# gotzmann/llama.go

Measured on AMD Instinct MI355X. Metric: decode tokens/s LLaMA-7B fp32; % HBM-read roofline, higher is better.
Workload: dtype f32

## Files before the change

llama.go_amd/csrc/kernels_common.h:

```cpp
#pragma once
#include <hip/hip_runtime.h>
#include <stdint.h>

namespace lh {

typedef float f4 __attribute__((ext_vector_type(4)));
typedef float f2 __attribute__((ext_vector_type(2)));
typedef unsigned int u4 __attribute__((ext_vector_type(4)));

struct StepParams {
    uint32_t token;
    uint32_t past;
    uint32_t step;
    uint32_t pad;
};

struct BatchRow {
    float* kc;
    float* vc;
    uint32_t pos;
    uint32_t step;
};

__device__ __forceinline__ f4 ld_nt(const f4* p) { return __builtin_nontemporal_load(p); }
// ... 31 lines not shown
}
__device__ __forceinline__ double wave_sum_f64(double v) {
#pragma unroll
    for (int o = 32; o >= 1; o >>= 1) v += __shfl_xor(v, o, 64);
    return v;
}

__device__ __forceinline__ void wg_row_block(uint32_t M, uint32_t wg_q, uint32_t wg_r, uint32_t* r0, uint32_t* r1) {
    const uint32_t b = blockIdx.x, nwg = gridDim.x;
    if (wg_q | wg_r) {
        *r0 = 2u * (b * wg_q + (b < wg_r ? b : wg_r));
        *r1 = (b + 1 == nwg) ? M : 2u * ((b + 1) * wg_q + (b + 1 < wg_r ? b + 1 : wg_r));
    } else {
        const uint32_t npairs = M >> 1;
        *r0 = 2u * (uint32_t)(((uint64_t)b * npairs) / nwg);
        *r1 = (b + 1 == nwg) ? M : 2u * (uint32_t)(((uint64_t)(b + 1) * npairs) / nwg);
    }
}

#define LH_TOUCH_ARGS(...) do { lh::touch_args_(__VA_ARGS__); } while (0)
template <typename A, typename B> __device__ __forceinline__ void touch_args_(A a, B b) { asm volatile("" ::"s"(a), "s"(b)); }
template <typename A, typename B, typename C> __device__ __forceinline__ void touch_args_(A a, B b, C c) { asm volatile("" ::"s"(a), "s"(b), "s"(c)); }
template <typename A, typename B, typename C, typename D> __device__ __forceinline__ void touch_args_(A a, B b, C c, D d) { asm volatile("" ::"s"(a), "s"(b), "s"(c), "s"(d)); }
template <typename A, typename B, typename C, typename D, typename E, typename F> __device__ __forceinline__ void touch_args_(A a, B b, C c, D d, E e, F f) {
    asm volatile("" ::"s"(a), "s"(b), "s"(c), "s"(d), "s"(e), "s"(f));
}

__device__ __forceinline__ const char* sgpr_ptr(const void* p) {
    uint32_t lo = (uint32_t)(uintptr_t)p, hi = (uint32_t)((uintptr_t)p >> 32);
    lo = __builtin_amdgcn_readfirstlane(lo);
    hi = __builtin_amdgcn_readfirstlane(hi);
    asm volatile("" : "+s"(lo), "+s"(hi));
    return (const char*)(((uintptr_t)hi << 32) | lo);
}

__device__ __forceinline__ float silu_ref(float x) {
    const float den = (float)(1.0 + exp((double)(-x)));
    return __fdiv_rn(x, den);
}
__device__ __forceinline__ void rope_rotate(float x0f, float x1f, double2 cs, float* o0, float* o1) {
    const double x0 = (double)x0f, x1 = (double)x1f;
    *o0 = (float)__dsub_rn(__dmul_rn(x0, cs.x), __dmul_rn(x1, cs.y));
    *o1 = (float)__dadd_rn(__dmul_rn(x0, cs.y), __dmul_rn(x1, cs.x));
}

__device__ __forceinline__ void split3(float x, uint32_t* hi, uint32_t* mid, uint32_t* lo) {
// ... 12 lines not shown
```

llama.go_amd/csrc/kernels_llama.h:

```cpp
#pragma once
#include "kernels_common.h"

namespace lh {

enum { PRO_PLAIN = 0, PRO_RMSNORM = 1 };
enum { EPI_STORE = 0, EPI_RESID = 1, EPI_QKV_ROPE = 2, EPI_SILU_MUL = 3 };
enum { MAP_SINGLE = 0, MAP_BLOCK = 1, MAP_PAIR = 2 };

struct GemvArgs {
    const float* w[3];
    const float* ws[3];
    uint32_t rows_per_mat;
    uint32_t M;
    uint32_t K;
    const float* x;
    const float* gamma;
    float* y;
    const float* resid;
    float* q_out;
    float* k_cache;
    float* v_cache;
    const double2* rope;
    uint32_t hd;
    uint32_t d;
    const StepParams* sp;
    uint32_t wg_q, wg_r;
};

template <int KI, int TH>
__device__ __forceinline__ void rmsnorm_prologue(f4 (&xr)[KI], const bool (&act)[KI], const f4 (&gr)[KI], uint32_t K, double* sred) {
    constexpr int NW = TH / 64;
    const int tid = threadIdx.x, lane = tid & 63, wave = tid >> 6;
    double s = 0.0;
#pragma unroll
    for (int j = 0; j < KI; ++j) {
        if (act[j]) {
            s += (double)__fmul_rn(xr[j].x, xr[j].x);
            s += (double)__fmul_rn(xr[j].y, xr[j].y);
            s += (double)__fmul_rn(xr[j].z, xr[j].z);
            s += (double)__fmul_rn(xr[j].w, xr[j].w);
        }
    }
    s = wave_sum_f64(s);
    if (lane == 0) sred[wave] = s;
    __syncthreads();
    double tot = 0.0;
#pragma unroll
    for (int w = 0; w < NW; ++w) tot += sred[w];
    const double mean = tot / (double)K;
    const float scale = (float)(1.0 / sqrt(mean + 1e-5));
#pragma unroll
    for (int j = 0; j < KI; ++j) {
        if (act[j]) {
            const f4 g = gr[j];
            xr[j].x = __fmul_rn(g.x, __fmul_rn(xr[j].x, scale));
            xr[j].y = __fmul_rn(g.y, __fmul_rn(xr[j].y, scale));
            xr[j].z = __fmul_rn(g.z, __fmul_rn(xr[j].z, scale));
            xr[j].w = __fmul_rn(g.w, __fmul_rn(xr[j].w, scale));
        }
    }
}

template <int EPI, int NP>
__device__ __forceinline__ void gemv_finish(const GemvArgs& a, const float* red, uint32_t r0, uint32_t r1, uint32_t fin, float resid_pre,
                                            double2 cs_pre, uint32_t past_pre) {
    if (r0 + fin >= r1) return;
    const float* p0 = red + fin * NP;
    float s0 = 0.f;
#pragma unroll
    for (int k = 0; k < NP; ++k) s0 += p0[k];
    const uint32_t v = r0 + fin;
    if (EPI == EPI_STORE) {
        a.y[v] = s0;
    } else if (EPI == EPI_RESID) {
        a.y[v] = __fadd_rn(s0, resid_pre);
    } else {
        const float* p1 = p0 + NP;
        float s1 = 0.f;
#pragma unroll
        for (int k = 0; k < NP; ++k) s1 += p1[k];
        if (EPI == EPI_SILU_MUL) {
            a.y[v >> 1] = __fmul_rn(silu_ref(s0), s1);
        } else {
            const uint32_t d = a.d;
// ... 24 lines not shown
    } else if (EPI == EPI_QKV_ROPE) {
        *past_pre = a.sp->past;
        const uint32_t v = r0 + fin;
        if (v < r1 && v < 2 * a.d) {
            const uint32_t e = v < a.d ? v : v - a.d;
            *cs_pre = a.rope[(size_t)*past_pre * (a.hd >> 1) + ((e % a.hd) >> 1)];
        }
    }
}

template <int MAP>
__device__ __forceinline__ const char* gemv_row_base(const char* w0, const char* w1, const char* w2, uint32_t rows_per_mat, uint32_t v, uint64_t row_bytes) {
    if (MAP == MAP_SINGLE) return w0 + (uint64_t)v * row_bytes;
    if (MAP == MAP_BLOCK) {
        const uint32_t m = (v >= rows_per_mat ? 1u : 0u) + (v >= 2u * rows_per_mat ? 1u : 0u);
        const char* b = m == 0 ? w0 : (m == 1 ? w1 : w2);
        return b + (uint64_t)(v - m * rows_per_mat) * row_bytes;
    }
    return ((v & 1u) ? w1 : w0) + (uint64_t)(v >> 1) * row_bytes;
}

template <int KI, int U, int TH, int PRO, int EPI, int MAP>
__global__ __launch_bounds__(TH) void k_gemv_sa(const GemvArgs a) {
    LH_TOUCH_ARGS(a.w[0], a.x, a.hd, a.wg_r);
    extern __shared__ __attribute__((aligned(16))) char smem_raw[];
    constexpr int NW = TH / 64;
    double* sred = (double*)smem_raw;
    float* red = (float*)(smem_raw + NW * 8);
    const int tid = threadIdx.x, lane = tid & 63, wave = tid >> 6;
    const uint32_t K4 = a.K >> 2;
    uint32_t r0, r1;
    wg_row_block(a.M, a.wg_q, a.wg_r, &r0, &r1);
    const char *w0 = (const char*)a.w[0], *w1 = (const char*)a.w[1], *w2 = (const char*)a.w[2];
    const char* xdummy = (const char*)a.x;
    const uint32_t rpm = a.rows_per_mat;
    const uint64_t row_bytes = (uint64_t)a.K * 4;

    const uint32_t fin = (EPI == EPI_STORE || EPI == EPI_RESID) ? (uint32_t)tid : 2u * (uint32_t)tid;
    float resid_pre;
    double2 cs_pre;
    uint32_t past_pre;
    gemv_prefetch_fin<EPI>(a, r0, r1, fin, &resid_pre, &cs_pre, &past_pre);
    f4 xr[KI];
    f4 gr[KI];
    bool act[KI];
    uint32_t loff[KI];
#pragma unroll
    for (int j = 0; j < KI; ++j) {
        act[j] = (uint32_t)(tid + j * TH) < K4;
        loff[j] = act[j] ? (uint32_t)(tid + j * TH) * 16u : 0u;
        xr[j] = act[j] ? ((const f4*)a.x)[tid + j * TH] : f4{0.f, 0.f, 0.f, 0.f};
        if (PRO == PRO_RMSNORM) gr[j] = act[j] ? ((const f4*)a.gamma)[tid + j * TH] : f4{0.f, 0.f, 0.f, 0.f};
    }
    f4 w[U][KI];
#pragma unroll
    for (int u = 0; u < U; ++u) {
        const char* p = (r0 + u < r1) ? gemv_row_base<MAP>(w0, w1, w2, rpm, r0 + u, row_bytes) : xdummy;
#pragma unroll
        for (int j = 0; j < KI; ++j) w[u][j] = ld_nt((const f4*)(p + loff[j]));
    }
    if (PRO == PRO_RMSNORM) rmsnorm_prologue<KI, TH>(xr, act, gr, a.K, sred);
    for (uint32_t r = r0; r < r1; r += U) {
        float acc[U];
#pragma unroll
        for (int u = 0; u < U; ++u) {
            const uint32_t nr = r + U + u;
            const char* p = nr < r1 ? gemv_row_base<MAP>(w0, w1, w2, rpm, nr, row_bytes) : xdummy;
            float s = 0.f;
#pragma unroll
            for (int j = 0; j < KI; ++j) {
                const f4 c = w[u][j];
                s = fmaf(c.x, xr[j].x, s);
                s = fmaf(c.y, xr[j].y, s);
                s = fmaf(c.z, xr[j].z, s);
                s = fmaf(c.w, xr[j].w, s);
                w[u][j] = ld_nt((const f4*)(p + loff[j]));
            }
            acc[u] = s;
        }
#pragma unroll
        for (int u = 0; u < U; ++u) acc[u] = wave_sum(acc[u]);
        if (lane == 0) {
#pragma unroll
            for (int u = 0; u < U; ++u)
// ... 234 lines not shown
    for (uint32_t t0 = ph + VP * phases; t0 < T; t0 += VP * phases) {
        float vv[VP];
#pragma unroll
        for (int i = 0; i < VP; ++i) {
            const uint32_t t = t0 + (uint32_t)i * phases;
            vv[i] = Vc[(size_t)(t < T ? t : 0) * d + c];
        }
#pragma unroll
        for (int i = 0; i < VP; ++i) {
            const uint32_t t = t0 + (uint32_t)i * phases;
            if (t < T) acc = fmaf(vv[i], __fmul_rn(pr[t], inv), acc);
        }
    }
    scratch[tid] = acc;
    __syncthreads();
    if (tid < (int)hd) {
        float o = scratch[tid];
        for (uint32_t p2 = 1; p2 < phases; ++p2) o += scratch[tid + p2 * hd];
        a.out[(size_t)j * d + h * hd + tid] = o;
        if (a.out_s3) attn_store_split3(a, (size_t)j * d + h * hd + tid, o);
    }
}

constexpr int ATT_TC = 128;

__global__ __launch_bounds__(ATT_TH) void k_attention_split(const AttnArgs a, float* __restrict__ part) {
    LH_TOUCH_ARGS(a.q, a.sp, a.rows);
    __shared__ float sc[ATT_TC];
    __shared__ float pr[ATT_TC];
    __shared__ float scratch[ATT_TH];
    constexpr int NG = ATT_TH / 32;
    const int tid = threadIdx.x, lane = tid & 63;
    const uint32_t h = blockIdx.x, ch = blockIdx.y, nch = gridDim.y, j = blockIdx.z;
    const uint32_t past = a.rows ? a.rows[j].pos : (a.sp ? a.sp->past : a.past_host);
    const uint32_t T = past + 1, c0 = ch * ATT_TC;
    if (c0 >= T) return;
    const uint32_t Tl = (T - c0 < (uint32_t)ATT_TC) ? T - c0 : (uint32_t)ATT_TC;
    const uint32_t d = a.d, hd = a.hd;
    const float* q = a.q + (size_t)j * d + h * hd;
    typedef const float __attribute__((address_space(1))) gfl;
    typedef const f4 __attribute__((address_space(1))) gf4;
    gfl* Kc = (gfl*)(uintptr_t)((a.rows ? a.rows[j].kc + a.kv_off : a.k_cache) + (size_t)c0 * d + h * hd);
    gfl* Vc = (gfl*)(uintptr_t)((a.rows ? a.rows[j].vc + a.kv_off : a.v_cache) + (size_t)c0 * d + h * hd);
    const uint32_t phases = ATT_TH / hd, c = tid % hd, ph = tid / hd;
    constexpr int VP = ATT_TC / 8;
    float vpre[VP];
#pragma unroll
    for (int i = 0; i < VP; ++i) {
// ... 312 lines not shown
```

llama.go_amd/csrc/kernels_q8.h:

```cpp
#pragma once
#include "kernels_llama.h"

namespace lh {

__device__ __forceinline__ u4 ld_nt_u4(const u4* p) { return __builtin_nontemporal_load(p); }


__device__ __forceinline__ float dot16_q8(const u4 q, const f4 (&x)[4]) {
    f2 a0 = {0.f, 0.f}, a1 = {0.f, 0.f};
#pragma unroll
    for (int k = 0; k < 4; ++k) {
        const int d = (int)q[k];
        const f2 w0 = {(float)(int)(signed char)(d), (float)(int)(signed char)(d >> 8)};
        const f2 w1 = {(float)(int)(signed char)(d >> 16), (float)(d >> 24)};
        a0 = __builtin_elementwise_fma(w0, f2{x[k].x, x[k].y}, a0);
        a1 = __builtin_elementwise_fma(w1, f2{x[k].z, x[k].w}, a1);
    }
    return (a0.x + a0.y) + (a1.x + a1.y);
}

template <int KI, int U, int TPR, int PRO, int EPI, int MAP, int TH = 1024>
__global__ __launch_bounds__(TH) void k_gemv_q8s(const GemvArgs a) {
    LH_TOUCH_ARGS(a.w[0], a.x, a.hd, a.wg_r);
    extern __shared__ __attribute__((aligned(16))) char smem_raw[];
    constexpr int G = TH / TPR, NWR = TPR / 64;
    static_assert(TPR % 64 == 0, "a row group must be a whole number of waves");
    double* sred = (double*)smem_raw;
    float* red = (float*)(smem_raw + 16 * 8);
    const int tid = threadIdx.x, lane = tid & 63, wave = tid >> 6;
    const int tr = tid % TPR, wr = wave % NWR;
    const uint32_t grp = (uint32_t)__builtin_amdgcn_readfirstlane(tid / TPR);
    const uint32_t K = a.K, K16 = K >> 4;
    uint32_t r0, r1;
    wg_row_block(a.M, a.wg_q, a.wg_r, &r0, &r1);
    const uint64_t q0 = (uint64_t)sgpr_ptr(a.w[0]), s0 = (uint64_t)sgpr_ptr(a.ws[0]);
    const uint64_t dq1 = MAP == MAP_SINGLE ? 0 : (uint64_t)sgpr_ptr(a.w[1]) - q0, ds1 = MAP == MAP_SINGLE ? 0 : (uint64_t)sgpr_ptr(a.ws[1]) - s0;
    const uint64_t dq2 = MAP == MAP_BLOCK ? (uint64_t)sgpr_ptr(a.w[2]) - q0 - dq1 : 0, ds2 = MAP == MAP_BLOCK ? (uint64_t)sgpr_ptr(a.ws[2]) - s0 - ds1 : 0;
    const uint64_t xdummy = (uint64_t)sgpr_ptr(a.x);
    const uint32_t rpm = a.rows_per_mat;
    const uint64_t srow = (uint64_t)(K >> 5) * 4u;
    const uint64_t e1q = dq1 - (uint64_t)rpm * K, e2q = dq2 - (uint64_t)rpm * K, e1s = ds1 - (uint64_t)rpm * srow, e2s = ds2 - (uint64_t)rpm * srow;
    const uint32_t mlo = (r0 >= rpm ? 1u : 0u) + (r0 >= 2u * rpm ? 1u : 0u), mhi = (r1 - 1u >= rpm ? 1u : 0u) + (r1 - 1u >= 2u * rpm ? 1u : 0u);
    const bool one_mat = mhi - mlo <= 1u;
    const uint64_t qv_wg = q0 + (mlo >= 1u ? e1q : 0) + (mlo == 2u ? e2q : 0), sv_wg = s0 + (mlo >= 1u ? e1s : 0) + (mlo == 2u ? e2s : 0);
    const uint32_t bnd = (mlo + 1u) * rpm;
    const uint64_t nq = (mlo == 0u ? e1q : 0) + (mlo == 1u ? e2q : 0), ns = (mlo == 0u ? e1s : 0) + (mlo == 1u ? e2s : 0);
    const uint32_t fin = (EPI == EPI_STORE || EPI == EPI_RESID) ? (uint32_t)tid : 2u * (uint32_t)tid;
    float resid_pre;
    double2 cs_pre;
    uint32_t past_pre;
    gemv_prefetch_fin<EPI>(a, r0, r1, fin, &resid_pre, &cs_pre, &past_pre);
    f4 xr[KI][4];
    bool act[KI];
    uint32_t qoff[KI], soff[KI];
#pragma unroll
    for (int j = 0; j < KI; ++j) {
        const uint32_t c = tr + j * TPR;
        act[j] = c < K16;
        qoff[j] = act[j] ? c * 16u : 0u;
        soff[j] = act[j] ? (c >> 1) * 4u : 0u;
#pragma unroll
        for (int k = 0; k < 4; ++k) xr[j][k] = act[j] ? ((const f4*)a.x)[c * 4 + k] : f4{0.f, 0.f, 0.f, 0.f};
    }
    f4 gr[PRO == PRO_RMSNORM ? KI : 1][4];
    if (PRO == PRO_RMSNORM) {
#pragma unroll
        for (int j = 0; j < KI; ++j)
#pragma unroll
            for (int k = 0; k < 4; ++k) gr[j][k] = act[j] ? ((const f4*)a.gamma)[(tr + j * TPR) * 4 + k] : f4{0.f, 0.f, 0.f, 0.f};
    }

    auto fetch = [&](u4 (&wd)[U][KI], float (&sd)[U][KI], uint32_t row_base) {
#pragma unroll
        for (int u = 0; u < U; ++u) {
            const uint32_t row = row_base + G * u;
            uint64_t qb = xdummy, sb = xdummy;
            if (MAP == MAP_BLOCK) {
                if (row < r1) {
                    uint64_t bq = qv_wg + (row >= bnd ? nq : 0), bs = sv_wg + (row >= bnd ? ns : 0);
                    if (!one_mat) {
                        bq = q0 + (row >= rpm ? e1q : 0) + (row >= 2u * rpm ? e2q : 0);
                        bs = s0 + (row >= rpm ? e1s : 0) + (row >= 2u * rpm ? e2s : 0);
                    }
                    qb = bq + (uint64_t)row * K;
                    sb = bs + (uint64_t)row * srow;
                }
            } else
            if (row < r1) {
                uint32_t m = 0, r = row;
                if (MAP == MAP_PAIR) { m = row & 1u; r = row >> 1; }
                qb = q0 + (m >= 1u ? dq1 : 0) + (uint64_t)r * K;
                sb = s0 + (m >= 1u ? ds1 : 0) + (uint64_t)r * srow;
            }
            typedef const u4 __attribute__((address_space(1))) gu4;
            typedef const float __attribute__((address_space(1))) gf32;
#pragma unroll
            for (int j = 0; j < KI; ++j) {
                wd[u][j] = __builtin_nontemporal_load((gu4*)(qb + qoff[j]));
                sd[u][j] = *(gf32*)(sb + soff[j]);
            }
        }
    };
    u4 wA[U][KI], wB[U][KI];
    float scA[U][KI], scB[U][KI];
    fetch(wA, scA, r0 + grp);
    constexpr uint32_t STEP = G * U;

    if (PRO == PRO_RMSNORM) {
        double s = 0.0;
#pragma unroll
        for (int j = 0; j < KI; ++j)
#pragma unroll
            for (int k = 0; k < 4; ++k) {
                if (act[j]) {
                    s += (double)__fmul_rn(xr[j][k].x, xr[j][k].x);
                    s += (double)__fmul_rn(xr[j][k].y, xr[j][k].y);
                    s += (double)__fmul_rn(xr[j][k].z, xr[j][k].z);
                    s += (double)__fmul_rn(xr[j][k].w, xr[j][k].w);
                }
            }
        s = wave_sum_f64(s);
        if (lane == 0) sred[wave] = s;
        __syncthreads();
        double tot = 0.0;
#pragma unroll
        for (int k = 0; k < NWR; ++k) tot += sred[grp * NWR + k];
        const float scale = (float)(1.0 / sqrt(tot / (double)K + 1e-5));
#pragma unroll
        for (int j = 0; j < KI; ++j)
#pragma unroll
// ... 42 lines not shown
```

llama.go_amd/csrc/plan.h:

```cpp
#pragma once
#include "common.h"
#include "kernels_common.h"
#include "attn_worklist.h"

namespace lh {

struct SampleState;

struct LayerW {
    const float *attn_norm = nullptr, *wq = nullptr, *wk = nullptr, *wv = nullptr, *wo = nullptr, *ffn_norm = nullptr, *w1 = nullptr, *w2 = nullptr, *w3 = nullptr;
    const float *s_wq = nullptr, *s_wk = nullptr, *s_wv = nullptr, *s_wo = nullptr, *s_w1 = nullptr, *s_w2 = nullptr, *s_w3 = nullptr;
    bool operator==(const LayerW& o) const {
        return attn_norm == o.attn_norm && wq == o.wq && wk == o.wk && wv == o.wv && wo == o.wo && ffn_norm == o.ffn_norm && w1 == o.w1 && w2 == o.w2 && w3 == o.w3;
    }
};

struct ModelDesc {
    uint32_t V = 0, d = 0, H = 0, hd = 0, L = 0, F = 0, ctx = 0;
    uint32_t layer0 = 0, layer1 = 0;
    uint32_t cache_layer0 = 0;
    const float *tok_emb = nullptr, *norm = nullptr, *output = nullptr;
    const float* s_output = nullptr;
    int wtype = 0;
    std::vector<LayerW> layers;
    float *kc = nullptr, *vc = nullptr;
    std::shared_ptr<std::vector<uint32_t>> kv_hist;
    bool same(const ModelDesc& o) const {
        return V == o.V && d == o.d && H == o.H && hd == o.hd && L == o.L && F == o.F && ctx == o.ctx && layer0 == o.layer0 && layer1 == o.layer1 &&
               cache_layer0 == o.cache_layer0 && wtype == o.wtype && tok_emb == o.tok_emb && norm == o.norm && output == o.output && kc == o.kc && vc == o.vc && layers == o.layers;
    }
    bool first_stage() const { return layer0 == 0; }
    bool last_stage() const { return layer1 == L; }
};

struct Plan {
    lh_ctx* ctx = nullptr;
    ModelDesc md;
    uint32_t n_cap = 0;
    uint64_t scratch_gen = 0;
    float *xa = nullptr, *xb = nullptr, *h = nullptr, *qraw = nullptr, *kraw = nullptr, *vraw = nullptr, *q = nullptr, *attn = nullptr;
    float *a1 = nullptr, *a3 = nullptr, *g = nullptr, *logits = nullptr;
    uint16_t* s3 = nullptr;
    uint32_t s3_rows = 0;
    float* emb = nullptr;
    uint32_t emb_cap = 0;
    float* attn_part = nullptr;
    float *scores = nullptr, *vt = nullptr;
    uint64_t scores_cap = 0, vt_cap = 0;
    float* part = nullptr;
    uint64_t part_cap = 0;
    float* fa_part = nullptr;
    uint64_t fa_part_cap = 0;
    FaWork fa_work;
    uint32_t* tokens_dev = nullptr;
    const double2* rope = nullptr;
    StepParams* sp_dev = nullptr;
    StepParams* sp_host = nullptr;
    uint32_t* out_tokens_dev = nullptr;
    uint32_t out_cap = 0;
    uint32_t* argmax_dev = nullptr;
    enum { G_STEP = 0, G_ADV1, G_ADVN, G_SMP1, G_SMPN, G_COUNT };
    static constexpr uint32_t GRAPH_MULTI = 8;
    hipGraph_t graph[G_COUNT] = {};
    hipGraphExec_t exec[G_COUNT] = {};
    struct SampleState* ss_dev = nullptr;
    uint32_t* ring_dev = nullptr;
    uint32_t ring_cap = 0;
    uint32_t smp_topk = 0;
    uint32_t slot_counter = 0;
// ... 37 lines not shown
```

llama.go_amd/csrc/plan.hip:

```cpp
#include "plan.h"
#include "kernels_llama.h"
#include "kernels_gemm.h"
#include "kernels_q8.h"
#include "kernels_skinny.h"
#include "kernels_attn.h"
#include "kernels_sample.h"
#include "kernels_stream.h"
#include "kernels_stream_q8b.h"
#include "kernels_stream_b9.h"
#include "kernels_gemm_b9.h"
#include "kernels_rows.h"
#include <math.h>
#include <string.h>
#include <algorithm>

namespace lh {

static thread_local bool g_prepare_only = false;
static thread_local const char* g_only = nullptr;
static inline bool skip_launch(const char* name) { return g_prepare_only || (g_only && strcmp(g_only, name) != 0); }

static constexpr int TH = 1024;
static constexpr size_t FAT_LDS = 96 * 1024;

// ... 75 lines not shown
    int rc = set_lds_once(ctx, k_gemv_q8s<KI, U, TPR, PRO, EPI, MAP, THR>, FAT_LDS, flags);
    if (rc) return rc;
    if (skip_launch(name)) return 0;
    ProfScope ps(ctx->stream, name, bytes);
    GemvArgs b = a;
    b.wg_q = (a.M / 2) / (uint32_t)ctx->ds->num_cu; b.wg_r = (a.M / 2) % (uint32_t)ctx->ds->num_cu;
    LH_LAUNCH((k_gemv_q8s<KI, U, TPR, PRO, EPI, MAP, THR>), dim3(ctx->ds->num_cu), dim3(THR), FAT_LDS, ctx->stream, b);
    LH_HIP(ctx, hipGetLastError());
    return 0;
}

template <int PRO, int EPI, int MAP>
static int gemv_q8(lh_ctx* ctx, const GemvArgs& a, const char* name) {
    if (a.K % 32 || ((EPI == EPI_QKV_ROPE || EPI == EPI_SILU_MUL) && a.M % 2))
        LH_FAIL(ctx, LH_ESHAPE, "gemv_q8 %s: K=%u must be a multiple of 32%s", name, a.K, a.M % 2 ? " and the row count even" : "");
    if ((uint64_t)a.M / ctx->ds->num_cu + 4 > (uint64_t)TH) LH_FAIL(ctx, LH_EUNSUPPORTED, "gemv_q8 %s: M=%u exceeds %d rows per workgroup", name, a.M, TH - 4);
    const uint32_t K16 = a.K / 16;
    const uint64_t bytes = (uint64_t)a.M * a.K / 32 * 36;
    const uint32_t rows_wg = a.M / (uint32_t)ctx->ds->num_cu;
    if (rows_wg + 4 <= 250) {
        if (K16 <= 256) return MAP == MAP_BLOCK ? launch_gemv_q8<1, 6, 256, PRO, EPI, MAP, 256>(ctx, a, name, bytes) : launch_gemv_q8<1, 4, 256, PRO, EPI, MAP, 256>(ctx, a, name, bytes);
        if (K16 > 512 && K16 <= 768) return launch_gemv_q8<3, 2, 256, PRO, EPI, MAP, 256>(ctx, a, name, bytes);
    }
    if (K16 <= 256) return rows_wg >= 32 ? launch_gemv_q8<1, 2, 256, PRO, EPI, MAP>(ctx, a, name, bytes) : launch_gemv_q8<1, 1, 256, PRO, EPI, MAP>(ctx, a, name, bytes);
    if (K16 <= 512) return launch_gemv_q8<2, 2, 256, PRO, EPI, MAP>(ctx, a, name, bytes);
    if (K16 <= 1024) return launch_gemv_q8<1, 2, 1024, PRO, EPI, MAP>(ctx, a, name, bytes);
    if (K16 <= 2048) return launch_gemv_q8<2, 2, 1024, PRO, EPI, MAP>(ctx, a, name, bytes);
    LH_FAIL(ctx, LH_EUNSUPPORTED, "gemv_q8 %s: K=%u exceeds the supported 32768 columns", name, a.K);
}

template <int PRO, int EPI, int MAP>
static int gemv_f32(lh_ctx* ctx, const GemvArgs& a, const char* name);

template <int PRO, int EPI, int MAP>
static int gemv(lh_ctx* ctx, const GemvArgs& a, const char* name, int wtype = 0) {
    return wtype == 7 ? gemv_q8<PRO, EPI, MAP>(ctx, a, name) : gemv_f32<PRO, EPI, MAP>(ctx, a, name);
}

template <int PRO, int EPI, int MAP>
static int gemv_f32(lh_ctx* ctx, const GemvArgs& a, const char* name) {
    if (a.K % 4 || ((EPI == EPI_QKV_ROPE || EPI == EPI_SILU_MUL) && a.M % 2))
        LH_FAIL(ctx, LH_ESHAPE, "gemv %s: K=%u must be a multiple of 4%s", name, a.K, a.M % 2 ? " and the row count even" : "");
    const uint32_t K4 = a.K / 4;
    const uint64_t bytes = (uint64_t)a.M * a.K * 4;
    const uint32_t rows_wg = a.M / (uint32_t)ctx->ds->num_cu + 4;
    if (K4 <= 4 * 256 && rows_wg <= 256) {
        switch ((K4 + 255) / 256) {
            case 1: return launch_gemv<1, 4, PRO, EPI, MAP, 256>(ctx, a, name, bytes);
            case 2: return launch_gemv<2, 4, PRO, EPI, MAP, 256>(ctx, a, name, bytes);
            case 3: return launch_gemv<3, 2, PRO, EPI, MAP, 256>(ctx, a, name, bytes);
            default: return launch_gemv<4, 2, PRO, EPI, MAP, 256>(ctx, a, name, bytes);
        }
    }
    if (K4 <= 6 * 512 && rows_wg <= 512) {
        switch ((K4 + 511) / 512) {
            case 1: return launch_gemv<1, 2, PRO, EPI, MAP, 512>(ctx, a, name, bytes);
            case 2: return launch_gemv<2, 2, PRO, EPI, MAP, 512>(ctx, a, name, bytes);
            case 3: return launch_gemv<3, 2, PRO, EPI, MAP, 512>(ctx, a, name, bytes);
            case 4: return launch_gemv<4, 1, PRO, EPI, MAP, 512>(ctx, a, name, bytes);
            case 5: return launch_gemv<5, 1, PRO, EPI, MAP, 512>(ctx, a, name, bytes);
            default: return launch_gemv<6, 1, PRO, EPI, MAP, 512>(ctx, a, name, bytes);
        }
    }
    if (rows_wg > (uint32_t)TH) LH_FAIL(ctx, LH_EUNSUPPORTED, "gemv %s: M=%u exceeds %d rows per workgroup", name, a.M, TH - 4);
    switch ((K4 + TH - 1) / TH) {
        case 1: return launch_gemv<1, 2, PRO, EPI, MAP>(ctx, a, name, bytes);
        case 2: return launch_gemv<2, 2, PRO, EPI, MAP>(ctx, a, name, bytes);
        case 3: return launch_gemv<3, 1, PRO, EPI, MAP>(ctx, a, name, bytes);
        case 4: return launch_gemv<4, 2, PRO, EPI, MAP>(ctx, a, name, bytes);
        case 5: return launch_gemv<5, 2, PRO, EPI, MAP>(ctx, a, name, bytes);
        case 6: return launch_gemv<6, (PRO == PRO_RMSNORM ? 1 : 2), PRO, EPI, MAP>(ctx, a, name, bytes);
        default: LH_FAIL(ctx, LH_EUNSUPPORTED, "gemv %s: K=%u exceeds the supported 24576 columns", name, a.K);
    }
}

template <int KI, int U, int THR, int NC, int PRO, int EPI, int MAP>
static int launch_gemv_rows(lh_ctx* ctx, const GemvRowsArgs& a, const char* name, uint64_t bytes) {
    static bool flags[16] = {};
    int rc = set_lds_once(ctx, k_gemv_rows<KI, U, THR, NC, PRO, EPI, MAP>, FAT_LDS, flags);
    if (rc) return rc;
    if (g_prepare_only) return 0;
    ProfScope ps(ctx->stream, name, bytes);
    GemvRowsArgs b = a;
    b.wg_q = (a.M / 2) / (uint32_t)ctx->ds->num_cu; b.wg_r = (a.M / 2) % (uint32_t)ctx->ds->num_cu;
    LH_LAUNCH((k_gemv_rows<KI, U, THR, NC, PRO, EPI, MAP>), dim3(ctx->ds->num_cu), dim3(THR), FAT_LDS, ctx->stream, b);
    LH_HIP(ctx, hipGetLastError());
    return 0;
}
static bool gemv_rows_shape_ok(lh_ctx* ctx, uint32_t M, uint32_t K, uint32_t nc = 4, bool norm = false) {
    const uint32_t K4 = K / 4, rows_wg = M / (uint32_t)ctx->ds->num_cu + 4;
    if (K % 4 || M % 2) return false;
    if (K4 <= 4 * 256 && rows_wg <= 256) return true;
    if (nc > 4 && (norm || K4 > 6 * 512)) return false;
    return K4 <= 6 * 512 && rows_wg <= 512;
}
template <int NC, int PRO, int EPI, int MAP>
// ... 847 lines not shown
    return 0;
}

static int launch_attention(lh_ctx* ctx, const AttnArgs& a, uint32_t max_T) {
    if (a.hd > ATT_TH || ATT_TH % a.hd || a.hd % 4) LH_FAIL(ctx, LH_EUNSUPPORTED, "attention: head dim %u unsupported (needs to divide %d)", a.hd, ATT_TH);
    const size_t lds = (2 * (size_t)((max_T + 63) & ~63u) + ATT_TH) * 4;
    static bool flags[16] = {};
    static size_t cur[16] = {};
    if (lds > 48 * 1024 && lds > cur[ctx->device & 15]) {
        flags[ctx->device & 15] = false;
        int rc = set_lds_once(ctx, k_attention, 160 * 1024, flags);
        if (rc) return rc;
        cur[ctx->device & 15] = 160 * 1024;
    }
    if (lds > 160 * 1024) LH_FAIL(ctx, LH_EUNSUPPORTED, "attention: %u keys exceed the single-pass LDS budget", max_T);
    if (g_prepare_only) return 0;
    if (g_only) return 0;
    ProfScope ps(ctx->stream, "attention", (uint64_t)2 * max_T * a.d * 4);
    LH_LAUNCH(k_attention, dim3(a.d / a.hd, a.n), dim3(ATT_TH), lds, ctx->stream, a);
    LH_HIP(ctx, hipGetLastError());
    return 0;
}

static int launch_attention_split(Plan* p, const AttnArgs& a, float* part) {
    lh_ctx* ctx = p->ctx;
    const ModelDesc& m = p->md;
    if (a.hd != 128) LH_FAIL(ctx, LH_EUNSUPPORTED, "split attention: head dim %u", a.hd);
    const uint32_t nch = (m.ctx + ATT_TC - 1) / ATT_TC, nrows = a.rows ? a.n : 1u;
    if (g_prepare_only || g_only) return 0;
    {
        ProfScope ps(ctx->stream, "attention_split", (uint64_t)2 * m.ctx * a.d * 4 * nrows);
        LH_LAUNCH(k_attention_split, dim3(m.H, nch, nrows), dim3(ATT_TH), 0, ctx->stream, a, part);
    }
    {
        ProfScope ps(ctx->stream, "attention_combine", (uint64_t)m.H * nch * (a.hd + 2) * 4 * nrows);
        LH_LAUNCH(k_attention_combine, dim3(m.H, nrows), dim3(128), 0, ctx->stream, a, (const float*)part, nch);
    }
    LH_HIP(ctx, hipGetLastError());
    return 0;
}

static void drop_graphs(Plan* p, uint32_t mask) {
    for (int i = 0; i < Plan::G_COUNT; ++i) {
        if (!(mask & (1u << i))) continue;
        if (p->exec[i]) { hipGraphExecDestroy(p->exec[i]); p->exec[i] = nullptr; }
        if (p->graph[i]) { hipGraphDestroy(p->graph[i]); p->graph[i] = nullptr; }
    }
}
static constexpr uint32_t GM_ADV = (1u << Plan::G_ADV1) | (1u << Plan::G_ADVN), GM_SMP = (1u << Plan::G_SMP1) | (1u << Plan::G_SMPN);

int plan_ensure_rows(Plan* p, uint32_t n) {
    if (n <= p->n_cap) return 0;
    lh_ctx* ctx = p->ctx;
    LH_HIP(ctx, hipStreamSynchronize(ctx->stream));
    const ModelDesc& m = p->md;
    auto re = [&](float** ptr, size_t nfloats) -> int {
        if (*ptr) LH_HIP(ctx, hipFree(*ptr));
// ... 23 lines not shown

static constexpr uint32_t SP_SLOTS = 64;

int plan_create(lh_ctx* ctx, const ModelDesc& md, Plan** out) {
    if (md.d % md.H || md.d % 4 || md.F % 4) LH_FAIL(ctx, LH_ESHAPE, "plan: embd %u / heads %u / ff %u not supported", md.d, md.H, md.F);
    Plan* p = new Plan();
    p->ctx = ctx;
    p->md = md;
    const char* env = getenv("LLAMAHIP_NO_GRAPH");
    p->use_graph = !(env && env[0] == '1');
    int rc = ensure_rope_table(ctx, md.ctx, md.hd, &p->rope);
    if (rc) { delete p; return rc; }
    hipError_t e = hipMalloc((void**)&p->sp_dev, sizeof(StepParams) * SP_SLOTS);
    if (e == hipSuccess) e = hipHostMalloc((void**)&p->sp_host, sizeof(StepParams) * SP_SLOTS, hipHostMallocDefault);
    if (e == hipSuccess) e = hipMalloc((void**)&p->argmax_dev, 4);
    if (e != hipSuccess) { set_error(ctx, "plan_create: %s", hipGetErrorString(e)); plan_destroy(p); return LH_ENOMEM; }
    rc = plan_ensure_rows(p, 1);
    if (rc) { plan_destroy(p); return rc; }
    p->hist = md.kv_hist ? md.kv_hist : std::make_shared<std::vector<uint32_t>>();
    if (p->hist->size() < md.ctx) p->hist->resize(md.ctx, Plan::HIST_UNKNOWN);
    if (md.ctx > 256 && md.hd == 128) {
        const size_t nch = (md.ctx + ATT_TC - 1) / ATT_TC;
        e = hipMalloc((void**)&p->attn_part, (size_t)md.H * nch * (md.hd + 2) * 4);
        if (e != hipSuccess) { set_error(ctx, "plan_create: %s", hipGetErrorString(e)); plan_destroy(p); return LH_ENOMEM; }
    }
    *out = p;
    return 0;
}

void plan_destroy(Plan* p) {
    if (!p) return;
    hipSetDevice(p->ctx->device);
    hipStreamSynchronize(p->ctx->stream);
    drop_graphs(p, ~0u);
    if (p->ss_dev) hipFree(p->ss_dev);
    if (p->ring_dev) hipFree(p->ring_dev);
    float* bufs[] = {p->xa, p->xb, p->h, p->qraw, p->kraw, p->vraw, p->q, p->attn, p->a1, p->a3, p->g, p->logits, p->scores, p->vt, p->part, p->fa_part, p->emb};
    for (float* b : bufs) if (b) hipFree(b);
    if (p->tokens_dev) hipFree(p->tokens_dev);
    if (p->sp_dev) hipFree(p->sp_dev);
    if (p->sp_host) hipHostFree(p->sp_host);
    if (p->out_tokens_dev) hipFree(p->out_tokens_dev);
    if (p->argmax_dev) hipFree(p->argmax_dev);
    if (p->attn_part) hipFree(p->attn_part);
    if (p->s3) hipFree(p->s3);
    delete p;
}
// ... 30 lines not shown
            TraceScope ts_(ctx->stream, "embed1");
            LH_LAUNCH(k_embed, dim3(1), dim3(256), 0, ctx->stream, m.tok_emb, tokens_dev, sp, p->xa, m.d, m.V);
            LH_HIP(ctx, hipGetLastError());
        }
    } else {
        x = x_in;
    }
    float* xa = p->xa;
    float* xb = p->xb;
    const float scale = (float)(1.0 / sqrt((double)m.d / (double)m.H));
    for (uint32_t il = m.layer0; il < m.layer1; ++il) {
        const LayerW& L = m.layers[il];
        const size_t slot = (size_t)(il - m.cache_layer0) * m.ctx * m.d;
        {
            GemvArgs a = {};
            a.w[0] = L.wq; a.w[1] = L.wk; a.w[2] = L.wv; a.ws[0] = L.s_wq; a.ws[1] = L.s_wk; a.ws[2] = L.s_wv; a.rows_per_mat = m.d; a.M = 3 * m.d; a.K = m.d;
            a.x = x; a.gamma = L.attn_norm; a.q_out = p->q; a.k_cache = m.kc + slot; a.v_cache = m.vc + slot;
            a.rope = rope; a.hd = m.hd; a.d = m.d; a.sp = sp;
            if ((rc = gemv<PRO_RMSNORM, EPI_QKV_ROPE, MAP_BLOCK>(ctx, a, "gemv_qkv_rope", m.wtype))) return rc;
        }
        {
            AttnArgs a = {};
            a.q = p->q; a.k_cache = m.kc + slot; a.v_cache = m.vc + slot; a.out = p->attn; a.d = m.d; a.hd = m.hd; a.n = 1; a.scale = scale; a.sp = sp;
            if (p->attn_part) { if ((rc = launch_attention_split(p, a, p->attn_part))) return rc; }
            else if ((rc = launch_attention(ctx, a, m.ctx))) return rc;
        }
        {
            GemvArgs a = {};
            a.w[0] = L.wo; a.ws[0] = L.s_wo; a.M = m.d; a.K = m.d; a.x = p->attn; a.resid = x; a.y = xb;
            if ((rc = gemv<PRO_PLAIN, EPI_RESID, MAP_SINGLE>(ctx, a, "gemv_wo_resid", m.wtype))) return rc;
        }
        {
            GemvArgs a = {};
            a.w[0] = L.w1; a.w[1] = L.w3; a.ws[0] = L.s_w1; a.ws[1] = L.s_w3; a.M = 2 * m.F; a.K = m.d; a.x = xb; a.gamma = L.ffn_norm; a.y = p->g;
            if ((rc = gemv<PRO_RMSNORM, EPI_SILU_MUL, MAP_PAIR>(ctx, a, "gemv_w1w3_silu", m.wtype))) return rc;
        }
        {
            const bool last = il + 1 == m.layer1;
            GemvArgs a = {};
            a.w[0] = L.w2; a.ws[0] = L.s_w2; a.M = m.d; a.K = m.F; a.x = p->g; a.resid = xb;
            a.y = (last && !m.last_stage()) ? x_out : xa;
            if ((rc = gemv<PRO_PLAIN, EPI_RESID, MAP_SINGLE>(ctx, a, "gemv_w2_resid", m.wtype))) return rc;
        }
        x = xa;
    }
    if (m.last_stage()) {
        {
            GemvArgs a = {};
            a.w[0] = m.output; a.ws[0] = m.s_output; a.M = m.V; a.K = m.d; a.x = x; a.gamma = m.norm; a.y = p->logits + logits_row * (size_t)m.V;
            if ((rc = gemv<PRO_RMSNORM, EPI_STORE, MAP_SINGLE>(ctx, a, "gemv_lmhead", m.wtype))) return rc;
        }
        if (g_only) {
// ... 1328 lines not shown
```

Measured before the change: 218.9.

## Fold split-attention combine into the Wo GEMV prologue

Removes the separate attention_combine kernel launch when the shape fits. Each workgroup of the Wo GEMV reads the per-chunk partial outputs and max/sum values, builds softmax weights in LDS and reduces the partials into its x vector. Weight loads are issued before this work so the two can overlap. The cost is that every workgroup redundantly recomputes the combine and reads all partials, which adds LDS use and a few barriers. It is gated by a chunk-count cap and shape checks.

```diff
diff --git a/llama.go_amd/csrc/kernels_common.h b/llama.go_amd/csrc/kernels_common.h
--- a/llama.go_amd/csrc/kernels_common.h
+++ b/llama.go_amd/csrc/kernels_common.h
@@ -77,6 +77,9 @@
 template <typename A, typename B> __device__ __forceinline__ void touch_args_(A a, B b) { asm volatile("" ::"s"(a), "s"(b)); }
 template <typename A, typename B, typename C> __device__ __forceinline__ void touch_args_(A a, B b, C c) { asm volatile("" ::"s"(a), "s"(b), "s"(c)); }
 template <typename A, typename B, typename C, typename D> __device__ __forceinline__ void touch_args_(A a, B b, C c, D d) { asm volatile("" ::"s"(a), "s"(b), "s"(c), "s"(d)); }
+template <typename A, typename B, typename C, typename D, typename E> __device__ __forceinline__ void touch_args_(A a, B b, C c, D d, E e) {
+    asm volatile("" ::"s"(a), "s"(b), "s"(c), "s"(d), "s"(e));
+}
 template <typename A, typename B, typename C, typename D, typename E, typename F> __device__ __forceinline__ void touch_args_(A a, B b, C c, D d, E e, F f) {
     asm volatile("" ::"s"(a), "s"(b), "s"(c), "s"(d), "s"(e), "s"(f));
 }
diff --git a/llama.go_amd/csrc/kernels_llama.h b/llama.go_amd/csrc/kernels_llama.h
--- a/llama.go_amd/csrc/kernels_llama.h
+++ b/llama.go_amd/csrc/kernels_llama.h
@@ -3,7 +3,7 @@
 
 namespace lh {
 
-enum { PRO_PLAIN = 0, PRO_RMSNORM = 1 };
+enum { PRO_PLAIN = 0, PRO_RMSNORM = 1, PRO_ATTN_COMBINE = 2 };
 enum { EPI_STORE = 0, EPI_RESID = 1, EPI_QKV_ROPE = 2, EPI_SILU_MUL = 3 };
 enum { MAP_SINGLE = 0, MAP_BLOCK = 1, MAP_PAIR = 2 };
 
@@ -25,6 +25,9 @@
     uint32_t d;
     const StepParams* sp;
     uint32_t wg_q, wg_r;
+    const float* att_part;
+    uint32_t att_nch;
+    uint32_t att_past;
 };
 
 template <int KI, int TH>
@@ -60,6 +63,117 @@
         }
     }
 }
+
+constexpr int ATT_TC = 128;
+constexpr int ATT_FOLD_HD = 128;
+constexpr int ATT_FOLD_LDS_OFF = 72 * 1024;
+constexpr int ATT_FOLD_LDS = 24 * 1024;
+constexpr int ATT_FOLD_ML = 4;
+constexpr int att_fold_pf(int nv) { return nv <= 4 ? 8 : (nv <= 8 ? 4 : 2); }
+
+template <int NV, int TH>
+struct AttnFold {
+    static constexpr int PF = att_fold_pf(NV), ML = ATT_FOLD_ML;
+    typedef f4 __attribute__((aligned(8))) f4p;
+    uint32_t n, lg;
+    uint32_t poff[NV];
+    uint32_t hh[NV];
+    f2 ml[ML];
+    f4 pv[PF][NV];
+
+    __device__ __forceinline__ void load(const GemvArgs& a, const uint32_t (&c4)[NV], const bool (&act)[NV]) {
+        const uint32_t past = a.sp ? a.sp->past : a.att_past;
+        const uint32_t nact = past / (uint32_t)ATT_TC + 1u;
+        n = nact < a.att_nch ? nact : a.att_nch;
+        lg = n > 1u ? 32u - (uint32_t)__builtin_clz(n - 1u) : 0u;
+        const uint32_t H = a.d / (uint32_t)ATT_FOLD_HD, st = ATT_FOLD_HD + 2, tid = threadIdx.x;
+#pragma unroll
+        for (int i = 0; i < ML; ++i) {
+            const uint32_t s = tid & ((1u << lg) - 1u), h = (tid >> lg) + (uint32_t)i * ((uint32_t)TH >> lg);
+            ml[i] = (s < n && h < H) ? *(const f2*)(a.att_part + ((size_t)h * a.att_nch + s) * st + ATT_FOLD_HD) : f2{0.f, 0.f};
+        }
+#pragma unroll
+        for (int v = 0; v < NV; ++v) {
+            hh[v] = act[v] ? (c4[v] * 4u) / (uint32_t)ATT_FOLD_HD : 0u;
+            poff[v] = hh[v] * a.att_nch * st + (act[v] ? (c4[v] * 4u) % (uint32_t)ATT_FOLD_HD : 0u);
+        }
+#pragma unroll
+        for (int s = 0; s < PF; ++s) {
+            if ((uint32_t)s < n) {
+#pragma unroll
+                for (int v = 0; v < NV; ++v) pv[s][v] = *(const f4p*)(a.att_part + poff[v] + (uint32_t)s * st);
+            } else {
+#pragma unroll
+                for (int v = 0; v < NV; ++v) pv[s][v] = f4{0.f, 0.f, 0.f, 0.f};
+            }
+        }
+    }
+
+    __device__ __forceinline__ void finish(const GemvArgs& a, f4 (&xr)[NV], const bool (&act)[NV], float* tab) {
+        const uint32_t H = a.d / (uint32_t)ATT_FOLD_HD, st = ATT_FOLD_HD + 2, tid = threadIdx.x;
+        float *cm = tab, *cl = tab + H * n, *cw = cl + H * n;
+        const uint32_t s = tid & ((1u << lg) - 1u), hstep = (uint32_t)TH >> lg;
+#pragma unroll
+        for (int i = 0; i < ML; ++i) {
+            const uint32_t h = (tid >> lg) + (uint32_t)i * hstep;
+            if (s < n && h < H) { cm[h * n + s] = ml[i].x; cl[h * n + s] = ml[i].y; }
+        }
+        if (s < n)
+            for (uint32_t h = (tid >> lg) + (uint32_t)ML * hstep; h < H; h += hstep) {
+                const f2 r = *(const f2*)(a.att_part + ((size_t)h * a.att_nch + s) * st + ATT_FOLD_HD);
+                cm[h * n + s] = r.x; cl[h * n + s] = r.y;
+            }
+        __syncthreads();
+        if (s < n)
+            for (uint32_t h = tid >> lg; h < H; h += hstep) {
+                float M = -INFINITY;
+                for (uint32_t t = 0; t < n; ++t) M = fmaxf(M, cm[h * n + t]);
+                cw[h * n + s] = (float)exp((double)__fsub_rn(cm[h * n + s], M));
+            }
+        __syncthreads();
+        float inv[NV];
+        f4 o[NV];
+#pragma unroll
+        for (int v = 0; v < NV; ++v) {
+            if (v > 0 && hh[v] == hh[v - 1]) {
+                inv[v] = inv[v - 1];
+            } else {
+                float l = 0.f;
+                for (uint32_t t = 0; t < n; ++t) l = fmaf(cl[hh[v] * n + t], cw[hh[v] * n + t], l);
+                inv[v] = __fdiv_rn(1.0f, l);
+            }
+            o[v] = f4{0.f, 0.f, 0.f, 0.f};
+        }
+        auto add = [&](const f4 (&pb)[PF][NV], uint32_t s0) {
+#pragma unroll
+            for (int u = 0; u < PF; ++u) {
+                if (s0 + (uint32_t)u < n) {
+#pragma unroll
+                    for (int v = 0; v < NV; ++v) {
+                        const float w = cw[hh[v] * n + s0 + (uint32_t)u];
+                        o[v].x = fmaf(pb[u][v].x, w, o[v].x); o[v].y = fmaf(pb[u][v].y, w, o[v].y);
+                        o[v].z = fmaf(pb[u][v].z, w, o[v].z); o[v].w = fmaf(pb[u][v].w, w, o[v].w);
+                    }
+                }
+            }
+        };
+        add(pv, 0);
+        for (uint32_t s0 = PF; s0 < n; s0 += PF) {
+#pragma unroll
+            for (int u = 0; u < PF; ++u) {
+                const uint32_t sc = s0 + (uint32_t)u < n ? s0 + (uint32_t)u : n - 1u;
+#pragma unroll
+                for (int v = 0; v < NV; ++v) pv[u][v] = *(const f4p*)(a.att_part + poff[v] + sc * st);
+            }
+            add(pv, s0);
+        }
+#pragma unroll
+        for (int v = 0; v < NV; ++v) {
+            xr[v].x = act[v] ? __fmul_rn(o[v].x, inv[v]) : 0.f; xr[v].y = act[v] ? __fmul_rn(o[v].y, inv[v]) : 0.f;
+            xr[v].z = act[v] ? __fmul_rn(o[v].z, inv[v]) : 0.f; xr[v].w = act[v] ? __fmul_rn(o[v].w, inv[v]) : 0.f;
+        }
+    }
+};
 
 template <int EPI, int NP>
 __device__ __forceinline__ void gemv_finish(const GemvArgs& a, const float* red, uint32_t r0, uint32_t r1, uint32_t fin, float resid_pre,
@@ -130,7 +244,8 @@
 
 template <int KI, int U, int TH, int PRO, int EPI, int MAP>
 __global__ __launch_bounds__(TH) void k_gemv_sa(const GemvArgs a) {
-    LH_TOUCH_ARGS(a.w[0], a.x, a.hd, a.wg_r);
+    if (PRO == PRO_ATTN_COMBINE) LH_TOUCH_ARGS(a.w[0], a.x, a.hd, a.sp, a.att_past);
+    else LH_TOUCH_ARGS(a.w[0], a.x, a.hd, a.wg_r);
     extern __shared__ __attribute__((aligned(16))) char smem_raw[];
     constexpr int NW = TH / 64;
     double* sred = (double*)smem_raw;
@@ -157,8 +272,15 @@
     for (int j = 0; j < KI; ++j) {
         act[j] = (uint32_t)(tid + j * TH) < K4;
         loff[j] = act[j] ? (uint32_t)(tid + j * TH) * 16u : 0u;
-        xr[j] = act[j] ? ((const f4*)a.x)[tid + j * TH] : f4{0.f, 0.f, 0.f, 0.f};
+        if (PRO != PRO_ATTN_COMBINE) xr[j] = act[j] ? ((const f4*)a.x)[tid + j * TH] : f4{0.f, 0.f, 0.f, 0.f};
         if (PRO == PRO_RMSNORM) gr[j] = act[j] ? ((const f4*)a.gamma)[tid + j * TH] : f4{0.f, 0.f, 0.f, 0.f};
+    }
+    AttnFold<KI, TH> fold;
+    if (PRO == PRO_ATTN_COMBINE) {
+        uint32_t c4[KI];
+#pragma unroll
+        for (int j = 0; j < KI; ++j) c4[j] = (uint32_t)(tid + j * TH);
+        fold.load(a, c4, act);
     }
     f4 w[U][KI];
 #pragma unroll
@@ -168,6 +290,7 @@
         for (int j = 0; j < KI; ++j) w[u][j] = ld_nt((const f4*)(p + loff[j]));
     }
     if (PRO == PRO_RMSNORM) rmsnorm_prologue<KI, TH>(xr, act, gr, a.K, sred);
+    if (PRO == PRO_ATTN_COMBINE) fold.finish(a, xr, act, (float*)(smem_raw + ATT_FOLD_LDS_OFF));
     for (uint32_t r = r0; r < r1; r += U) {
         float acc[U];
 #pragma unroll
@@ -448,8 +571,6 @@
     }
 }
 
-constexpr int ATT_TC = 128;
-
 __global__ __launch_bounds__(ATT_TH) void k_attention_split(const AttnArgs a, float* __restrict__ part) {
     LH_TOUCH_ARGS(a.q, a.sp, a.rows);
     __shared__ float sc[ATT_TC];
diff --git a/llama.go_amd/csrc/kernels_q8.h b/llama.go_amd/csrc/kernels_q8.h
--- a/llama.go_amd/csrc/kernels_q8.h
+++ b/llama.go_amd/csrc/kernels_q8.h
@@ -21,7 +21,8 @@
 
 template <int KI, int U, int TPR, int PRO, int EPI, int MAP, int TH = 1024>
 __global__ __launch_bounds__(TH) void k_gemv_q8s(const GemvArgs a) {
-    LH_TOUCH_ARGS(a.w[0], a.x, a.hd, a.wg_r);
+    if (PRO == PRO_ATTN_COMBINE) LH_TOUCH_ARGS(a.w[0], a.x, a.hd, a.sp, a.att_past);
+    else LH_TOUCH_ARGS(a.w[0], a.x, a.hd, a.wg_r);
     extern __shared__ __attribute__((aligned(16))) char smem_raw[];
     constexpr int G = TH / TPR, NWR = TPR / 64;
     static_assert(TPR % 64 == 0, "a row group must be a whole number of waves");
@@ -60,7 +61,18 @@
         qoff[j] = act[j] ? c * 16u : 0u;
         soff[j] = act[j] ? (c >> 1) * 4u : 0u;
 #pragma unroll
-        for (int k = 0; k < 4; ++k) xr[j][k] = act[j] ? ((const f4*)a.x)[c * 4 + k] : f4{0.f, 0.f, 0.f, 0.f};
+        for (int k = 0; k < 4; ++k)
+            if (PRO != PRO_ATTN_COMBINE) xr[j][k] = act[j] ? ((const f4*)a.x)[c * 4 + k] : f4{0.f, 0.f, 0.f, 0.f};
+    }
+    AttnFold<4 * KI, TH> fold;
+    bool act4[4 * KI];
+    if (PRO == PRO_ATTN_COMBINE) {
+        uint32_t c4[4 * KI];
+#pragma unroll
+        for (int j = 0; j < KI; ++j)
+#pragma unroll
+            for (int k = 0; k < 4; ++k) { c4[j * 4 + k] = (tr + j * TPR) * 4 + k; act4[j * 4 + k] = act[j]; }
+        fold.load(a, c4, act4);
     }
     f4 gr[PRO == PRO_RMSNORM ? KI : 1][4];
     if (PRO == PRO_RMSNORM) {
@@ -106,6 +118,14 @@
     fetch(wA, scA, r0 + grp);
     constexpr uint32_t STEP = G * U;
 
+    if (PRO == PRO_ATTN_COMBINE) {
+        f4 xf[4 * KI];
+        fold.finish(a, xf, act4, (float*)(smem_raw + ATT_FOLD_LDS_OFF));
+#pragma unroll
+        for (int j = 0; j < KI; ++j)
+#pragma unroll
+            for (int k = 0; k < 4; ++k) xr[j][k] = xf[j * 4 + k];
+    }
     if (PRO == PRO_RMSNORM) {
         double s = 0.0;
 #pragma unroll
diff --git a/llama.go_amd/csrc/plan.h b/llama.go_amd/csrc/plan.h
--- a/llama.go_amd/csrc/plan.h
+++ b/llama.go_amd/csrc/plan.h
@@ -45,6 +45,7 @@
     float* emb = nullptr;
     uint32_t emb_cap = 0;
     float* attn_part = nullptr;
+    bool att_fold = false;
     float *scores = nullptr, *vt = nullptr;
     uint64_t scores_cap = 0, vt_cap = 0;
     float* part = nullptr;
diff --git a/llama.go_amd/csrc/plan.hip b/llama.go_amd/csrc/plan.hip
--- a/llama.go_amd/csrc/plan.hip
+++ b/llama.go_amd/csrc/plan.hip
@@ -121,11 +121,14 @@
         if (K16 <= 256) return MAP == MAP_BLOCK ? launch_gemv_q8<1, 6, 256, PRO, EPI, MAP, 256>(ctx, a, name, bytes) : launch_gemv_q8<1, 4, 256, PRO, EPI, MAP, 256>(ctx, a, name, bytes);
         if (K16 > 512 && K16 <= 768) return launch_gemv_q8<3, 2, 256, PRO, EPI, MAP, 256>(ctx, a, name, bytes);
     }
+    if constexpr (PRO == PRO_ATTN_COMBINE) LH_FAIL(ctx, LH_ESHAPE, "gemv_q8 %s: %u x %u has no combine-prologue instantiation", name, a.M, a.K);
+    else {
     if (K16 <= 256) return rows_wg >= 32 ? launch_gemv_q8<1, 2, 256, PRO, EPI, MAP>(ctx, a, name, bytes) : launch_gemv_q8<1, 1, 256, PRO, EPI, MAP>(ctx, a, name, bytes);
     if (K16 <= 512) return launch_gemv_q8<2, 2, 256, PRO, EPI, MAP>(ctx, a, name, bytes);
     if (K16 <= 1024) return launch_gemv_q8<1, 2, 1024, PRO, EPI, MAP>(ctx, a, name, bytes);
     if (K16 <= 2048) return launch_gemv_q8<2, 2, 1024, PRO, EPI, MAP>(ctx, a, name, bytes);
     LH_FAIL(ctx, LH_EUNSUPPORTED, "gemv_q8 %s: K=%u exceeds the supported 32768 columns", name, a.K);
+    }
 }
 
 template <int PRO, int EPI, int MAP>
@@ -161,6 +164,8 @@
             default: return launch_gemv<6, 1, PRO, EPI, MAP, 512>(ctx, a, name, bytes);
         }
     }
+    if constexpr (PRO == PRO_ATTN_COMBINE) LH_FAIL(ctx, LH_ESHAPE, "gemv %s: %u x %u has no combine-prologue instantiation", name, a.M, a.K);
+    else {
     if (rows_wg > (uint32_t)TH) LH_FAIL(ctx, LH_EUNSUPPORTED, "gemv %s: M=%u exceeds %d rows per workgroup", name, a.M, TH - 4);
     switch ((K4 + TH - 1) / TH) {
         case 1: return launch_gemv<1, 2, PRO, EPI, MAP>(ctx, a, name, bytes);
@@ -171,6 +176,22 @@
         case 6: return launch_gemv<6, (PRO == PRO_RMSNORM ? 1 : 2), PRO, EPI, MAP>(ctx, a, name, bytes);
         default: LH_FAIL(ctx, LH_EUNSUPPORTED, "gemv %s: K=%u exceeds the supported 24576 columns", name, a.K);
     }
+    }
+}
+
+static constexpr uint32_t ATT_FOLD_MAX_CHUNKS = 256;
+static constexpr uint32_t ATT_FOLD_CHUNKS_F32 = 16, ATT_FOLD_CHUNKS_Q8 = 8;
+static_assert(ATT_FOLD_LDS_OFF + ATT_FOLD_LDS <= (int)FAT_LDS, "the fold's tables lie inside the fat workgroup's LDS request");
+static bool att_fold_shape_ok(lh_ctx* ctx, const ModelDesc& m) {
+    static const int cap_env = getenv("LLAMAHIP_ATT_FOLD") ? atoi(getenv("LLAMAHIP_ATT_FOLD")) : -1;
+    const uint32_t cap = cap_env >= 0 ? std::min((uint32_t)cap_env, ATT_FOLD_MAX_CHUNKS) : (m.wtype == 7 ? ATT_FOLD_CHUNKS_Q8 : ATT_FOLD_CHUNKS_F32);
+    if (m.hd != (uint32_t)ATT_FOLD_HD || m.d != m.H * m.hd) return false;
+    const uint32_t nch = (m.ctx + ATT_TC - 1) / ATT_TC, ncu = (uint32_t)ctx->ds->num_cu;
+    if (nch > cap || (size_t)3 * m.H * nch * 4 > (size_t)ATT_FOLD_LDS) return false;
+    if (m.wtype == 7) return m.d % 32 == 0 && m.d / ncu + 4 <= 250 && (m.d / 16 <= 256 || (m.d / 16 > 512 && m.d / 16 <= 768));
+    if (m.wtype != 0) return false;
+    const uint32_t K4 = m.d / 4, rows_wg = m.d / ncu + 4;
+    return (K4 <= 4 * 256 && rows_wg <= 256) || (K4 <= 6 * 512 && rows_wg <= 512);
 }
 
 template <int KI, int U, int THR, int NC, int PRO, int EPI, int MAP>
@@ -1064,7 +1085,7 @@
     return 0;
 }
 
-static int launch_attention_split(Plan* p, const AttnArgs& a, float* part) {
+static int launch_attention_split(Plan* p, const AttnArgs& a, float* part, bool combine = true) {
     lh_ctx* ctx = p->ctx;
     const ModelDesc& m = p->md;
     if (a.hd != 128) LH_FAIL(ctx, LH_EUNSUPPORTED, "split attention: head dim %u", a.hd);
@@ -1074,7 +1095,7 @@
         ProfScope ps(ctx->stream, "attention_split", (uint64_t)2 * m.ctx * a.d * 4 * nrows);
         LH_LAUNCH(k_attention_split, dim3(m.H, nch, nrows), dim3(ATT_TH), 0, ctx->stream, a, part);
     }
-    {
+    if (combine) {
         ProfScope ps(ctx->stream, "attention_combine", (uint64_t)m.H * nch * (a.hd + 2) * 4 * nrows);
         LH_LAUNCH(k_attention_combine, dim3(m.H, nrows), dim3(128), 0, ctx->stream, a, (const float*)part, nch);
     }
@@ -1144,7 +1165,9 @@
     if (md.ctx > 256 && md.hd == 128) {
         const size_t nch = (md.ctx + ATT_TC - 1) / ATT_TC;
         e = hipMalloc((void**)&p->attn_part, (size_t)md.H * nch * (md.hd + 2) * 4);
+        if (e == hipSuccess) e = hipMemset(p->attn_part, 0, (size_t)md.H * nch * (md.hd + 2) * 4);
         if (e != hipSuccess) { set_error(ctx, "plan_create: %s", hipGetErrorString(e)); plan_destroy(p); return LH_ENOMEM; }
+        p->att_fold = att_fold_shape_ok(ctx, md);
     }
     *out = p;
     return 0;
@@ -1221,12 +1244,16 @@
         {
             AttnArgs a = {};
             a.q = p->q; a.k_cache = m.kc + slot; a.v_cache = m.vc + slot; a.out = p->attn; a.d = m.d; a.hd = m.hd; a.n = 1; a.scale = scale; a.sp = sp;
-            if (p->attn_part) { if ((rc = launch_attention_split(p, a, p->attn_part))) return rc; }
+            if (p->attn_part) { if ((rc = launch_attention_split(p, a, p->attn_part, !p->att_fold))) return rc; }
             else if ((rc = launch_attention(ctx, a, m.ctx))) return rc;
         }
         {
             GemvArgs a = {};
             a.w[0] = L.wo; a.ws[0] = L.s_wo; a.M = m.d; a.K = m.d; a.x = p->attn; a.resid = x; a.y = xb;
+            if (p->att_fold) {
+                a.att_part = p->attn_part; a.att_nch = (m.ctx + ATT_TC - 1) / ATT_TC; a.sp = sp; a.hd = m.hd; a.d = m.d;
+                if ((rc = gemv<PRO_ATTN_COMBINE, EPI_RESID, MAP_SINGLE>(ctx, a, "gemv_wo_resid", m.wtype))) return rc;
+            } else
             if ((rc = gemv<PRO_PLAIN, EPI_RESID, MAP_SINGLE>(ctx, a, "gemv_wo_resid", m.wtype))) return rc;
         }
         {
```

After: 221.0 (median of 6 runs). No clear change (+0.9%).
